# nttcslab-sp/torchain

Hardware: AMD Instinct MI355X
Metric: sequence-frames/sec through denominator fwd-bwd (higher is better)
Workload: dtype f32

## Files before the change

### torchain_amd/csrc/den_tied_device.h

```cpp
#pragma once

#include "den_device.h"

namespace tc {

namespace {

typedef float f4 __attribute__((ext_vector_type(4)));
typedef uint32_t u4 __attribute__((ext_vector_type(4)));
typedef __attribute__((address_space(3))) float lds_f;
typedef __attribute__((address_space(3))) uint32_t lds_u;
typedef __attribute__((address_space(3))) f4 lds_f4;
typedef __attribute__((address_space(3))) u4 lds_u4;

__device__ __forceinline__ float ldsf(uint32_t a) { return *reinterpret_cast<lds_f *>(a); }
__device__ __forceinline__ void ldsf_st(uint32_t a, float v) { *reinterpret_cast<lds_f *>(a) = v; }
__device__ __forceinline__ f4 lds4(uint32_t a) { return *reinterpret_cast<lds_f4 *>(a); }
__device__ __forceinline__ void lds4_st(uint32_t a, f4 v) { *reinterpret_cast<lds_f4 *>(a) = v; }
__device__ __forceinline__ void lds4_st_at(uint32_t base, uint32_t off, f4 v) {
  asm volatile("ds_write_b128 %0, %1 offset:%2" : : "v"(base), "v"(v), "i"(off) : "memory");
}
__device__ __forceinline__ u4 lds4u(uint32_t a) { return *reinterpret_cast<lds_u4 *>(a); }
__device__ __forceinline__ void lds_add_u32(uint32_t a, uint32_t v) {
  __hip_atomic_fetch_add(reinterpret_cast<lds_u *>(a), v, __ATOMIC_RELAXED, __HIP_MEMORY_SCOPE_WORKGROUP);
}

typedef __amdgpu_buffer_rsrc_t rsrc_t;
__device__ __forceinline__ rsrc_t make_rsrc(const void *ubase, uint32_t bytes) {
  return __builtin_amdgcn_make_buffer_rsrc(const_cast<void *>(ubase), 0, (int)bytes, 0x00020000);
}
__device__ __forceinline__ u4 bld4u(rsrc_t r, uint32_t voff, uint32_t soff) {
  return __builtin_amdgcn_raw_buffer_load_b128(r, (int)voff, (int)soff, 0);
}
__device__ __forceinline__ f4 bld4(rsrc_t r, uint32_t voff, uint32_t soff) {
  const u4 v = bld4u(r, voff, soff);
  return f4{__uint_as_float(v.x), __uint_as_float(v.y), __uint_as_float(v.z), __uint_as_float(v.w)};
}
template <int AUX>
__device__ __forceinline__ f4 bld4_aux(rsrc_t r, uint32_t voff, uint32_t soff) {
  const u4 v = __builtin_amdgcn_raw_buffer_load_b128(r, (int)voff, (int)soff, AUX);
  return f4{__uint_as_float(v.x), __uint_as_float(v.y), __uint_as_float(v.z), __uint_as_float(v.w)};
}
__device__ __forceinline__ void bst4(rsrc_t r, uint32_t voff, f4 v) {
#ifndef TC_STORE_AUX
#define TC_STORE_AUX 2
#endif
  __builtin_amdgcn_raw_buffer_store_b128(u4{__float_as_uint(v.x), __float_as_uint(v.y), __float_as_uint(v.z), __float_as_uint(v.w)},
                                         r, (int)voff, 0, TC_STORE_AUX);
}

template <int AUX>
__device__ __forceinline__ void bst4_aux(rsrc_t r, uint32_t voff, f4 v) {
  __builtin_amdgcn_raw_buffer_store_b128(u4{__float_as_uint(v.x), __float_as_uint(v.y), __float_as_uint(v.z), __float_as_uint(v.w)},
                                         r, (int)voff, 0, AUX);
}

__device__ __forceinline__ f4 mk4(float x) { return f4{x, x, x, x}; }
__device__ __forceinline__ float hsum(f4 v) { return (v.x + v.y) + (v.z + v.w); }
__device__ __forceinline__ float exp_med3(float x) { return __expf(__builtin_amdgcn_fmed3f(x, -30.0f, 30.0f)); }
__device__ __forceinline__ f4 exp4(f4 y) { return f4{exp_med3(y.x), exp_med3(y.y), exp_med3(y.z), exp_med3(y.w)}; }

__device__ __forceinline__ f4 row_ld(rsrc_t r, uint32_t voff, int vec) {
  if (vec) return bld4(r, voff, 0);
  return f4{__uint_as_float(__builtin_amdgcn_raw_buffer_load_b32(r, (int)voff, 0, 0)),
            __uint_as_float(__builtin_amdgcn_raw_buffer_load_b32(r, (int)voff, 4, 0)),
            __uint_as_float(__builtin_amdgcn_raw_buffer_load_b32(r, (int)voff, 8, 0)),
            __uint_as_float(__builtin_amdgcn_raw_buffer_load_b32(r, (int)voff, 12, 0))};
}
__device__ __forceinline__ void row_st(rsrc_t r, uint32_t voff, int vec, f4 v) {
  if (vec) {
    bst4(r, voff, v);
  } else {
    __builtin_amdgcn_raw_buffer_store_b32(__float_as_uint(v.x), r, (int)voff, 0, 0);
    __builtin_amdgcn_raw_buffer_store_b32(__float_as_uint(v.y), r, (int)voff, 4, 0);
    __builtin_amdgcn_raw_buffer_store_b32(__float_as_uint(v.z), r, (int)voff, 8, 0);
    __builtin_amdgcn_raw_buffer_store_b32(__float_as_uint(v.w), r, (int)voff, 12, 0);
  }
}

__device__ __forceinline__ float block_sum_a(float v, uint32_t red, int wave, uint32_t lane) {
  v = wave_sum(v);
  if (lane == 0) ldsf_st(red + 4u * (uint32_t)wave, v);
  __syncthreads();
  static_assert(kWaves == 16, "one DPP row holds the wave totals");
  float t = ldsf(red + 4u * (lane & 15u));
  t = dpp_add<0xB1>(t);
  t = dpp_add<0x4E>(t);
  t = dpp_add<0x124>(t);
  t = dpp_add<0x128>(t);
  return t;
}

__device__ __forceinline__ void gamma_add_a(uint32_t addr, float v) {
  int32_t q;
  asm("v_cvt_rpi_i32_f32 %0, %1" : "=v"(q) : "v"(v));
  lds_add_u32(addr, (uint32_t)q);
}

struct Chunk6 {
  u4 wa, wb, oc;
};

__device__ __forceinline__ void load_chunk(Chunk6 &q, rsrc_t stream, uint32_t lane16, int chunk) {
  const uint32_t so = (uint32_t)chunk * (3 * 64 * 16);
  q.wa = bld4u(stream, lane16, so);
  q.wb = bld4u(stream, lane16, so + 1024);
  q.oc = bld4u(stream, lane16, so + 2048);
}

__device__ __forceinline__ uint32_t lo16(uint32_t x) {
  uint32_t r;
  asm volatile("v_and_b32 %0, 0xffff, %1" : "=v"(r) : "v"(x));
  return r;
}
__device__ __forceinline__ uint32_t hi16(uint32_t x) {
  uint32_t r;
  asm volatile("v_lshrrev_b32 %0, 16, %1" : "=v"(r) : "v"(x));
  return r;
}

__device__ __forceinline__ uint32_t lo16w(uint32_t x) {
  uint32_t r;
  const uint32_t two = 2u;
  asm volatile("v_lshlrev_b32_sdwa %0, %1, %2 dst_sel:DWORD dst_unused:UNUSED_PAD src0_sel:DWORD src1_sel:WORD_0" : "=v"(r) : "s"(two), "v"(x));
  return r;
}
__device__ __forceinline__ uint32_t hi16w(uint32_t x) {
  uint32_t r;
  const uint32_t two = 2u;
  asm volatile("v_lshlrev_b32_sdwa %0, %1, %2 dst_sel:DWORD dst_unused:UNUSED_PAD src0_sel:DWORD src1_sel:WORD_1" : "=v"(r) : "s"(two), "v"(x));
  return r;
}

struct RowCommit {
  uint32_t row;
  uint32_t sec_row;
  int left;
  __device__ __forceinline__ void commit(float v) {
    asm volatile("s_mov_b32 m0, %1\n\ts_nop 0\n\tds_write_addtid_b32 %0" : : "v"(v), "s"(row) : "memory", "m0");
    --left;
    row = left == 0 ? sec_row : row + 256u;
  }
};

template <uint32_t SRC, int HALF>
__device__ __forceinline__ void do_chunk(const Chunk6 &q, uint32_t m, float &acc, RowCommit &rc) {
  uint32_t o[8];
  o[0] = lo16(q.oc.x);
  o[1] = hi16(q.oc.x);
  o[2] = lo16(q.oc.y);
  o[3] = hi16(q.oc.y);
  o[4] = lo16(q.oc.z);
  o[5] = hi16(q.oc.z);
  o[6] = lo16(q.oc.w);
  o[7] = hi16(q.oc.w);
  float a[8];
#pragma unroll
  for (int i = 0; i < 8; ++i) {
#ifdef TC_ABL_NOGATHER
    a[i] = __uint_as_float(o[i]);
#else
    a[i] = ldsf(SRC + o[i]);
#endif
  }
  const uint32_t w[8] = {q.wa.x, q.wa.y, q.wa.z, q.wa.w, q.wb.x, q.wb.y, q.wb.z, q.wb.w};
#pragma unroll
  for (int i = 0; i < 8; ++i) {
    acc = fmaf(a[i], __uint_as_float(w[i]), acc);
    const int bit = (i & 1) ? 4 * HALF + i / 2 : 8 + 4 * HALF + i / 2;
    if (__builtin_expect((m >> bit) & 1u, 0)) {
      rc.commit(acc);
      acc = 0.f;
    }
  }
}

__device__ __forceinline__ uint32_t wave_masks(const ScheduleDev &sc, int wave, uint32_t lane) {
  const uint32_t i = lane < (uint32_t)sc.mask_stride ? lane : (uint32_t)sc.mask_stride - 1u;
  return sc.masks[(size_t)wave * sc.mask_stride + i];
}

constexpr int kWalkEnd = -1000;

template <uint32_t SRC, int RES, class AfterChunk>
__device__ __forceinline__ void walk(const Chunk6 (&res)[RES > 0 ? RES : 1], Chunk6 &qa, rsrc_t sbase,
                                     uint32_t lane16, int nchunks, uint32_t vmask, RowCommit rc,
                                     AfterChunk after_chunk TC_WALK_ARG) {
  static_assert(RES % 2 == 0, "a mask word covers two chunks");
  auto mk = [&](int i) { return (uint32_t)__builtin_amdgcn_readlane((int)vmask, i); };
  float acc = 0.f;
#ifdef TC_PHASE_STAMPS
  wst[2] = clock64();
#endif
#pragma unroll
  for (int i = 0; i < RES / 2; ++i) {
    const uint32_t m = mk(i);
    do_chunk<SRC, 0>(res[2 * i], m, acc, rc);
    after_chunk(2 * i);
    do_chunk<SRC, 1>(res[2 * i + 1], m, acc, rc);
    after_chunk(2 * i + 1);
  }
#ifdef TC_PHASE_STAMPS
  {
    __builtin_amdgcn_s_waitcnt(0xC07F);
    const long long now = clock64();
    wst[0] += now - wst[2];
    wst[2] = now;
  }
#endif
  Chunk6 qb;
  int c = RES;
  for (; c + 2 < nchunks; c += 2) {
    const uint32_t m = mk(c >> 1);
    load_chunk(qb, sbase, lane16, c + 1);
    do_chunk<SRC, 0>(qa, m, acc, rc);
    load_chunk(qa, sbase, lane16, c + 2);
    do_chunk<SRC, 1>(qb, m, acc, rc);
    if (RES == 0) after_chunk(-1 - (c >> 1));
  }
  if (c + 1 < nchunks) {
    const uint32_t m = mk(c >> 1);
    load_chunk(qb, sbase, lane16, c + 1);
    do_chunk<SRC, 0>(qa, m, acc, rc);
    do_chunk<SRC, 1>(qb, m, acc, rc);
  } else if (c < nchunks) {
    do_chunk<SRC, 0>(qa, mk(c >> 1), acc, rc);
  }
  if (RES == 0) after_chunk(kWalkEnd);
#ifdef TC_PHASE_STAMPS
  __builtin_amdgcn_s_waitcnt(0xC07F);
  wst[1] += clock64() - wst[2];
#endif
}

template <uint32_t SRC>
__device__ __forceinline__ void chunk_pw(const Chunk6 &q, uint32_t m8, float &acc, RowCommit &rc) {
  uint32_t o[8];
  o[0] = lo16w(q.oc.x);
  o[1] = hi16w(q.oc.x);
  o[2] = lo16w(q.oc.y);
  o[3] = hi16w(q.oc.y);
  o[4] = lo16w(q.oc.z);
  o[5] = hi16w(q.oc.z);
  o[6] = lo16w(q.oc.w);
  o[7] = hi16w(q.oc.w);
  float a[8];
#pragma unroll
  for (int i = 0; i < 8; ++i) a[i] = ldsf(SRC + o[i]);
  const uint32_t w[8] = {q.wa.x, q.wa.y, q.wa.z, q.wa.w, q.wb.x, q.wb.y, q.wb.z, q.wb.w};
#pragma unroll
  for (int i = 0; i < 8; ++i) {
    acc = fmaf(a[i], __uint_as_float(w[i]), acc);
    if (__builtin_expect((m8 >> i) & 1u, 0)) {
      rc.commit(acc);
      acc = 0.f;
    }
  }
}

__device__ __forceinline__ void age_prio_on(int wave) {
  if (wave >= 12)
    __builtin_amdgcn_s_setprio(3);
  else if (wave >= 8)
    __builtin_amdgcn_s_setprio(2);
  else if (wave >= 4)
    __builtin_amdgcn_s_setprio(1);
}

__device__ __forceinline__ float tied_alpha(uint32_t pb, uint32_t fs, float ws, float F, float a_self) {
  return fmaf(ldsf(pb + (fs & 0xffffu)), F, ldsf(pb + (fs >> 16)) * (ws * a_self));
}

__device__ __forceinline__ f4 own_rows(uint32_t vrow, int j) {
  return f4{ldsf(vrow + 256u * (4 * j)), ldsf(vrow + 256u * (4 * j + 1)), ldsf(vrow + 256u * (4 * j + 2)),
            ldsf(vrow + 256u * (4 * j + 3))};
}

__device__ __forceinline__ void fold_row(int2 f, uint32_t vrow, uint32_t aACC, int Hs, int K) {
  const int k = 4 * (f.x / (4 * kThreads)) + (f.x & 3);
  const uint32_t dst = vrow + 256u * (uint32_t)k;
  const uint32_t src = aACC + 256u * (uint32_t)(K * kWaves) + 4u * (uint32_t)(f.y - Hs - 4);
  ldsf_st(dst, ldsf(dst) + ldsf(src));
}

__device__ __forceinline__ void fold_row_pw(int2 f, uint32_t vrow, uint32_t aACC, int Hs) {
  const uint32_t dst = vrow + 256u * (uint32_t)(f.x & 3);
  const uint32_t src = aACC + 256u * (uint32_t)(4 * kWaves) + 4u * (uint32_t)(f.y - Hs - 4);
  ldsf_st(dst, ldsf(dst) + ldsf(src));
}

constexpr uint32_t kPlane = 16u * kThreads;

struct AsumRow {
  uint32_t lds;
  float *g;
  __device__ __forceinline__ AsumRow(const DenParams &p, int s)
      : lds(4u * (uint32_t)p.L.off_asum), g(p.L.asum_global ? p.asum_g + (int64_t)s * asum_stride(p.T) : nullptr) {}
  __device__ __forceinline__ void st(int t, float v) const {
    if (g)
      g[t] = v;
    else
      ldsf_st(lds + 4u * (uint32_t)t, v);
  }
  __device__ __forceinline__ float ld(int t) const {
    if (g) return __uint_as_float(__builtin_amdgcn_raw_buffer_load_b32(make_rsrc(g + t, 4u), 0, 0, 0));
    return ldsf(lds + 4u * (uint32_t)t);
  }
};

}

#define TC_TIED_DISPATCH(CALL)                            \
  if (JV == kJvSmall && PV == kPvSmall) return CALL(kJvSmall, kPvSmall); \
  if (JV == kJvSmall && PV == kPvMid) return CALL(kJvSmall, kPvMid);     \
  if (JV == kJvSmall && PV == kPvLarge) return CALL(kJvSmall, kPvLarge); \
  if (JV == kJvMid && PV == kPvSmall) return CALL(kJvMid, kPvSmall);     \
  if (JV == kJvMid && PV == kPvMid) return CALL(kJvMid, kPvMid);         \
  if (JV == kJvMid && PV == kPvLarge) return CALL(kJvMid, kPvLarge);     \
  if (JV == kJvLarge && PV == kPvSmall) return CALL(kJvLarge, kPvSmall); \
  if (JV == kJvLarge && PV == kPvMid) return CALL(kJvLarge, kPvMid);     \
  if (JV == kJvLarge && PV == kPvLarge) return CALL(kJvLarge, kPvLarge);

}
```

### torchain_amd/csrc/den_tied_frames.h

```cpp
#pragma once

#include <type_traits>

#include "den_tied_device.h"

namespace tc {

__device__ __forceinline__ void block_sum2(float &v1, float &v2, uint32_t red, int wave, uint32_t lane) {
  v1 = wave_sum(v1);
  v2 = wave_sum(v2);
  if (lane == 0) {
    ldsf_st(red + 4u * (uint32_t)wave, v1);
    ldsf_st(red + 4u * (uint32_t)(kWaves + wave), v2);
  }
  __syncthreads();
  float t1 = ldsf(red + 4u * (lane & 15u)), t2 = ldsf(red + 4u * (kWaves + (lane & 15u)));
  t1 = dpp_add<0xB1>(t1);
  t2 = dpp_add<0xB1>(t2);
  t1 = dpp_add<0x4E>(t1);
  t2 = dpp_add<0x4E>(t2);
  t1 = dpp_add<0x124>(t1);
  t2 = dpp_add<0x124>(t2);
  v1 = dpp_add<0x128>(t1);
  v2 = dpp_add<0x128>(t2);
}

__device__ __forceinline__ float vload_f32(const float *ptr) {
  return __uint_as_float(__builtin_amdgcn_raw_buffer_load_b32(make_rsrc(ptr, 4u), 0, 0, 0));
}

template <bool GAMMA>
__device__ __forceinline__ float tied_fwd_state(uint32_t pb, uint32_t aGM, float inv_prev, uint32_t fsx, float wsx, float Fx, float alx,
                                                float bx, float gs, float &dpart) {
  const float pf = ldsf(pb + (fsx & 0xffffu)), ps = ldsf(pb + (fsx >> 16));
  const float sp = ps * (wsx * alx);
  const float a = fmaf(pf, Fx, sp) * inv_prev;
  if constexpr (GAMMA) {
    const float g = gs * bx, spn = sp * inv_prev;
    gamma_add_a(aGM + (fsx >> 16), g * spn);
    gamma_add_a(aGM + (fsx & 0xffffu), g * fmaxf(a - spn, 0.f));
    dpart = fmaf(a, bx, dpart);
  }
  return a;
}
template <bool PURE>
__device__ __forceinline__ float tied_bwd_state(uint32_t pb, uint32_t aGM, uint32_t fsx, float wsx, float bo, float alx, float aupx,
                                                float cpx, float ax, float inv_as, float asum_up) {
  const float ps_ws = ldsf(pb + (fsx >> 16)) * wsx;
  if constexpr (!PURE) {
    const float selfpart = ps_ws * alx * inv_as;
    const float bos = kGammaScale * bo;
    gamma_add_a(aGM + (fsx >> 16), bos * selfpart);
#ifndef TC_ABL_NOFADD
    gamma_add_a(aGM + (fsx & 0xffffu), bos * fmaxf((aupx - cpx * asum_up) - selfpart, 0.f));
#endif
  }
  return fmaf(ps_ws, bo, ax);
}

template <int JV, int PV, bool ALPHA_LDS, bool ACCUM, int RESF, int RESB, bool MITM>
struct TiedSeq {
  const DenParams &p;
  const uint32_t tid, lane;
  const int wave, s;
  const int H, P, S, T, Hs, Ps;
  const int planes, K;
  const uint32_t own16, lane16;
  static constexpr uint32_t kPB = 0u;
  static constexpr uint32_t kA0 = PV * 16u * kThreads;
  const uint32_t aACC;
  const uint32_t vrow;
  const uint32_t aGM;
  const uint32_t aAL;
  const uint32_t aRed, aAsum;
  const uint32_t tab_bytes, row_bytes;
  const rsrc_t r_pi, r_fs, r_ws;
  const float leaky;
  const int64_t hist_step;
  float *const hist;
  float *const fn;
  float *const bn;
  float *const bhist;
  const int M;

  int fnch, store_slot, bnch, bstore_slot;
  uint32_t fsec, bsec;
  uint32_t aFS, aWS;
  bool tabs_lds;
  uint32_t pb_cur, pb_next;
  rsrc_t fbase, bbase;
  float asum, inv_prev, bsum;
  float chat;
  float part, y2, part_tot;
  int ffx0, ffx1, bfx0, bfx1;
  uint32_t fmask, bmask;
  Chunk6 fres[RESF > 0 ? RESF : 1];
  Chunk6 bres[RESB > 0 ? RESB : 1];
  f4 v4[JV];
  f4 bt[JV];
  f4 areg[JV];
  f4 ycur[PV], ynext[PV];
  f4 bown[JV];
#ifdef TC_PHASE_STAMPS
  long long st_prev, st_acc[8];
#endif

  __device__ __forceinline__ TiedSeq(const DenParams &pp, int seq, int meet, int frames = 0)
      : p(pp), tid(threadIdx.x), lane(threadIdx.x & 63u), wave(__builtin_amdgcn_readfirstlane(threadIdx.x >> 6)), s(seq),
        H(pp.H), P(pp.P), S(pp.S), T(frames > 0 ? frames : pp.T), Hs(pp.L.Hs), Ps(pp.L.Ps), planes(pp.L.Hs / (4 * kThreads)), K(pp.L.Hs / kThreads),
        own16(16u * threadIdx.x), lane16(16u * (threadIdx.x & 63u)), aACC(4u * (uint32_t)pp.L.off_acc),
        vrow(4u * (uint32_t)pp.L.off_acc + 256u * (uint32_t)((pp.L.Hs / kThreads) * __builtin_amdgcn_readfirstlane(threadIdx.x >> 6)) +
             4u * (threadIdx.x & 63u)),
        aGM(4u * (uint32_t)pp.L.off_g), aAL(4u * (uint32_t)pp.L.off_al), aRed(4u * (uint32_t)pp.L.off_red),
        aAsum(4u * (uint32_t)pp.L.off_asum), tab_bytes(4u * (uint32_t)(pp.L.Hs + 4)), row_bytes(4u * (uint32_t)pp.P),
        r_pi(make_rsrc(pp.pi, 4u * (uint32_t)(pp.L.Hs + 4))), r_fs(make_rsrc(pp.tied_fs, 4u * (uint32_t)(pp.L.Hs + 4))),
        r_ws(make_rsrc(pp.tied_w, 4u * (uint32_t)(pp.L.Hs + 4))), leaky(pp.leaky), hist_step((int64_t)pp.S * pp.L.Hs),
        hist(pp.alpha_hist + (int64_t)seq * pp.L.Hs), fn(MITM ? pp.fwd_norm + (int64_t)seq * (pp.T + 2) : nullptr),
        bn(MITM ? pp.bwd_norm + (int64_t)seq * (pp.T + 1) : nullptr), bhist(MITM ? pp.beta_hist + (int64_t)seq * pp.L.Hs : nullptr),
        M(meet) {}

  __device__ __forceinline__ bool plane_on(int j) const { return j < planes; }

  __device__ __forceinline__ void stamps_reset() {
#ifdef TC_PHASE_STAMPS
    st_prev = clock64();
    for (int i = 0; i < 8; ++i) st_acc[i] = 0;
#endif
  }
  __device__ __forceinline__ void stamps_flush(int base) {
#ifdef TC_PHASE_STAMPS
    TC_STAMP(0)
    if (!MITM && blockIdx.x == 0 && lane == 0)
      for (int i = 0; i < 8; ++i) p.stamps[base + wave * 8 + i] = st_acc[i];
#endif
  }

  __device__ __forceinline__ void xent_zero_row(int t) {
    if (p.xent_zero) {
      const rsrc_t xrow = make_rsrc(p.xent_zero + ((int64_t)t * S + s) * p.xent_stride, row_bytes);
#pragma unroll
      for (int v = 0; v < PV; ++v)
        if (4 * ((int)tid + kThreads * v) < Ps) row_st(xrow, own16 + v * kPlane, p.x_vec, mk4(0.f));
    }
  }

  template <bool GAMMA>
  __device__ __forceinline__ float fwd_state(uint32_t fsx, float wsx, float Fx, float alx, float bx, float gs, float &dpart) {
    return tied_fwd_state<GAMMA>(kPB, aGM, inv_prev, fsx, wsx, Fx, alx, bx, gs, dpart);
  }
  template <bool PURE>
  __device__ __forceinline__ float bwd_state(uint32_t pb, uint32_t fsx, float wsx, float bo, float alx, float aupx, float cpx, float ax,
                                             float inv_as, float asum_up) {
    return tied_bwd_state<PURE>(pb, aGM, fsx, wsx, bo, alx, aupx, cpx, ax, inv_as, asum_up);
  }

  __device__ __forceinline__ void forward_begin() {
    f4 pi4[JV];
    part = 0.f;
#pragma unroll
    for (int j = 0; j < JV; ++j) {
      pi4[j] = plane_on(j) ? bld4(r_pi, own16, j * kPlane) : mk4(0.f);
      part += hsum(pi4[j]);
    }
    asum = block_sum_a(part, aRed, wave, lane);
#pragma unroll
    for (int j = 0; j < JV; ++j)
      if (plane_on(j)) {
        const f4 a = pi4[j] + (leaky * pi4[j]) * asum;
        lds4_st(kA0 + own16 + j * kPlane, a);
        bst4(make_rsrc(hist, 4u * Hs), own16 + j * kPlane, a);
      }
    y2 = 0.f;
    {
      const rsrc_t yrow = make_rsrc(p.y + (int64_t)s * p.y_stride, row_bytes);
#pragma unroll
      for (int v = 0; v < PV; ++v) {
        const int i0 = 4 * ((int)tid + kThreads * v);
        if (i0 < Ps) {
          const f4 yv = row_ld(yrow, own16 + v * kPlane, p.y_vec);
          y2 += hsum(yv * yv);
          lds4_st(kPB + 4u * i0, exp4(yv));
        }
      }
    }
    if (tid == 0) {
      ldsf_st(aAsum, asum);
      if (MITM) fn[0] = asum;
    }
    inv_prev = __builtin_amdgcn_rcpf(asum);

    {
    const int2 frange = p.fwd.wave_range[wave];
#ifdef TC_ABL_NOSTREAM
    fnch = RESF;
#else
    fnch = __builtin_amdgcn_readfirstlane(frange.y) / kChunk;
#endif
    fbase = make_rsrc(reinterpret_cast<const char *>(p.fwd.cells) +
                          (int64_t)(__builtin_amdgcn_readfirstlane(frange.x) / kChunk) * (3 * 64 * 16),
                      (uint32_t)(fnch + 2) * (3 * 64 * 16));
    fmask = wave_masks(p.fwd, wave, lane);
    ffx0 = p.fwd.nfix ? p.fwd.fix_begin[tid] : 0;
    ffx1 = p.fwd.nfix ? p.fwd.fix_begin[tid + 1] : 0;
    fsec = aACC + 256u * (uint32_t)(K * kWaves + p.fwd.extra_first[wave]);
#pragma unroll
    for (int i = 0; i < RESF; ++i) load_chunk(fres[i], fbase, lane16, i);
    }
    tabs_lds = (p.L.off_red - p.L.off_g) >= 2 * Hs;
    aFS = aGM;
    aWS = aGM + 4u * (uint32_t)Hs;
    if (tabs_lds) {
#pragma unroll
      for (int j = 0; j < JV; ++j)
        if (plane_on(j)) {
          *reinterpret_cast<lds_u4 *>(aFS + own16 + j * kPlane) = bld4u(r_fs, own16, j * kPlane);
          lds4_st(aWS + own16 + j * kPlane, bld4(r_ws, own16, j * kPlane));
        }
    }
    store_slot = RESF >= 4 ? wave >> 2 : RESF >= 2 ? wave >> 3 : 0;
#pragma unroll
    for (int j = 0; j < JV; ++j) v4[j] = bt[j] = mk4(0.f);
    chat = 0.f;
    part_tot = 0.f;
    stamps_reset();
  }

  static constexpr bool kHistFromPass = !MITM;

  template <bool GAMMA>
  __device__ __forceinline__ void forward_frame(int t) {
#ifdef TC_PHASE_STAMPS
    long long *const wst = st_acc + 5;
#endif
    TC_STAMP(0)
    Chunk6 q0;
    load_chunk(q0, fbase, lane16, RESF);
    __syncthreads();
    TC_STAMP(1)
    f4 yreg[PV];
    if (t < T) {
      const rsrc_t yrow = make_rsrc(p.y + ((int64_t)t * S + s) * p.y_stride, row_bytes);
#pragma unroll
      for (int v = 0; v < PV; ++v) yreg[v] = row_ld(yrow, own16 + v * kPlane, p.y_vec);
    }
    float n_t = 1.f;
    if (GAMMA && t < T) n_t = vload_f32(bn + t);
    age_prio_on(wave);
    bool stored = false;
    const RowCommit frc{aACC + 256u * (uint32_t)(K * wave), fsec, K};
    walk<kA0, RESF>(fres, q0, fbase, lane16, fnch, fmask, frc, [&](int i) {
      if (!kHistFromPass && !GAMMA && t > 1 && !stored && (RESF > 0 ? i == store_slot : (i == kWalkEnd || i == -1 - (wave >> 2)))) {
        stored = true;
        const rsrc_t hist_prev = make_rsrc(hist + (int64_t)(t - 1) * hist_step, 4u * Hs);
#ifndef TC_ABL_NOHIST
#pragma unroll
        for (int j = 0; j < JV; ++j)
          if (plane_on(j)) bst4(hist_prev, own16 + j * kPlane, lds4(kA0 + own16 + j * kPlane));
#endif
      }
    } TC_WALK_PASS);
    __builtin_amdgcn_s_setprio(0);
    TC_STAMP(2)
    for (int e = ffx0; e < ffx1; ++e) fold_row(p.fwd.fix[e], vrow, aACC, Hs, K);
    TC_STAMP(3)
    part = 0.f;
    float dpart = 0.f;
    u4 fs[JV];
    f4 ws[JV], cpi[JV];
#pragma unroll
    for (int j = 0; j < JV; ++j)
      if (plane_on(j)) {
        fs[j] = tabs_lds ? lds4u(aFS + own16 + j * kPlane) : bld4u(r_fs, own16, j * kPlane);
        ws[j] = tabs_lds ? lds4(aWS + own16 + j * kPlane) : bld4(r_ws, own16, j * kPlane);
        cpi[j] = bld4(r_pi, own16, j * kPlane);
      }
    const float gs = kGammaScale * chat;
    const rsrc_t hist_prev = make_rsrc(hist + (int64_t)(t - 1) * hist_step, t > 1 ? 4u * Hs : 0u);
#pragma unroll
    for (int j = 0; j < JV; ++j) {
      v4[j] = mk4(0.f);
      if (plane_on(j)) {
        const f4 F = own_rows(vrow, j);
        const f4 al = lds4(kA0 + own16 + j * kPlane);
#ifndef TC_ABL_NOHIST
        if (kHistFromPass && !GAMMA) bst4(hist_prev, own16 + j * kPlane, al);
#endif
        v4[j] = f4{fwd_state<GAMMA>(fs[j].x, ws[j].x, F.x, al.x, bt[j].x, gs, dpart), fwd_state<GAMMA>(fs[j].y, ws[j].y, F.y, al.y, bt[j].y, gs, dpart),
                   fwd_state<GAMMA>(fs[j].z, ws[j].z, F.z, al.z, bt[j].z, gs, dpart), fwd_state<GAMMA>(fs[j].w, ws[j].w, F.w, al.w, bt[j].w, gs, dpart)};
        part += hsum(v4[j]);
      }
    }
    f4 yp[PV];
    if (GAMMA) {
      const rsrc_t yprev = make_rsrc(p.y + ((int64_t)(t - 1) * S + s) * p.y_stride, row_bytes);
#pragma unroll
      for (int v = 0; v < PV; ++v) yp[v] = row_ld(yprev, own16 + v * kPlane, p.y_vec);
      const rsrc_t brow = make_rsrc(bhist + (int64_t)(t + 1 <= T ? t + 1 : T) * hist_step, 4u * Hs);
#pragma unroll
      for (int j = 0; j < JV; ++j) bt[j] = bld4(brow, own16, j * kPlane);
      block_sum2(part, dpart, aRed, wave, lane);
      asum = part;
    } else {
      asum = block_sum_a(part, aRed, wave, lane);
    }
    __builtin_amdgcn_sched_barrier(0);
    TC_STAMP(4)
    part_tot = 0.f;
#pragma unroll
    for (int j = 0; j < JV; ++j)
      if (plane_on(j)) {
        const f4 a = v4[j] + (leaky * cpi[j]) * asum;
        lds4_st(kA0 + own16 + j * kPlane, a);
        part_tot += hsum(a);
      }
    if (GAMMA) {
      const float c = __builtin_amdgcn_rcpf(dpart);
      const float sa = p.deriv_weight * (kGammaInvScale * (c * __builtin_amdgcn_rcpf(chat)));
      const rsrc_t drow = make_rsrc(p.deriv + ((int64_t)(t - 1) * S + s) * p.deriv_stride, row_bytes);
#pragma unroll
      for (int v = 0; v < PV; ++v) {
        const int i0 = 4 * ((int)tid + kThreads * v);
        if (i0 < Ps) {
          const u4 gu = lds4u(aGM + 4u * i0);
          lds4_st(aGM + 4u * i0, mk4(0.f));
          f4 o = sa * f4{(float)gu.x, (float)gu.y, (float)gu.z, (float)gu.w} - p.l2_scale * yp[v];
          if (ACCUM) o += row_ld(drow, own16 + v * kPlane, p.d_vec);
          row_st(drow, own16 + v * kPlane, p.d_vec, o);
        }
      }
      xent_zero_row(t - 1);
      chat = c * asum * __builtin_amdgcn_rcpf(n_t);
    }
    if (t < T) {
#pragma unroll
      for (int v = 0; v < PV; ++v) {
        const int i0 = 4 * ((int)tid + kThreads * v);
        if (i0 < Ps) {
          y2 += hsum(yreg[v] * yreg[v]);
          lds4_st(kPB + 4u * i0, exp4(yreg[v]));
        }
      }
    }
    if (tid == 0) {
      ldsf_st(aAsum + 4u * t, asum);
      if (MITM) fn[t] = asum;
    }
    inv_prev = __builtin_amdgcn_rcpf(asum);
  }

  __device__ __forceinline__ void forward_unpark() {
    tabs_lds = false;
#pragma unroll
    for (int v = 0; v < PV; ++v) {
      const int i0 = 4 * ((int)tid + kThreads * v);
      if (i0 < Ps) lds4_st(aGM + 4u * i0, mk4(0.f));
    }
  }

  __device__ __forceinline__ void forward_store_row(int t) {
    const rsrc_t hist_t = make_rsrc(hist + (int64_t)t * hist_step, 4u * Hs);
#pragma unroll
    for (int j = 0; j < JV; ++j)
      if (plane_on(j)) bst4(hist_t, own16 + j * kPlane, lds4(kA0 + own16 + j * kPlane));
  }

  __device__ __forceinline__ float forward_total(double bad) {
    const float tot = block_sum_a(part_tot, aRed + 4u * kWaves, wave, lane);
    const double y2d = (double)block_sum_a(y2, aRed + 8u * kWaves, wave, lane);
    if (tid == 0) {
      double logsum = 0.0;
      for (int t = 0; t < T; ++t) logsum += (double)__logf(ldsf(aAsum + 4u * t));
      p.seq_logprob[s] = logsum + (double)__logf(tot) + (y2d - y2d) + bad;
      p.seq_y2[s] = y2d;
    }
    return tot;
  }

  __device__ __forceinline__ void backward_store_row(int t) {
    const rsrc_t brow = make_rsrc(bhist + (int64_t)t * hist_step, 4u * Hs);
#pragma unroll
    for (int j = 0; j < JV; ++j)
      if (plane_on(j)) bst4(brow, own16 + j * kPlane, bown[j]);
  }

  template <bool PURE>
  __device__ __forceinline__ void backward_begin(float b_T) {
    part = 0.f;
#pragma unroll
    for (int j = 0; j < JV; ++j)
      if (plane_on(j)) part += hsum(leaky * bld4(r_pi, own16, j * kPlane)) * b_T;
    bsum = block_sum_a(part, aRed + 12u * kWaves, wave, lane);
    pb_cur = kPB;
    pb_next = ALPHA_LDS ? 4u * (uint32_t)p.L.off_p2 : kPB;
    {
    const int2 brange = p.bwd.wave_range[wave];
#ifdef TC_ABL_NOSTREAM
    bnch = RESB;
#else
    bnch = __builtin_amdgcn_readfirstlane(brange.y) / kChunk;
#endif
    bbase = make_rsrc(reinterpret_cast<const char *>(p.bwd.cells) +
                          (int64_t)(__builtin_amdgcn_readfirstlane(brange.x) / kChunk) * (3 * 64 * 16),
                      (uint32_t)(bnch + 2) * (3 * 64 * 16));
    bmask = wave_masks(p.bwd, wave, lane);
    bfx0 = p.bwd.nfix ? p.bwd.fix_begin[tid] : 0;
    bfx1 = p.bwd.nfix ? p.bwd.fix_begin[tid + 1] : 0;
    bsec = aACC + 256u * (uint32_t)(K * kWaves + p.bwd.extra_first[wave]);
#pragma unroll
    for (int i = 0; i < RESB; ++i) load_chunk(bres[i], bbase, lane16, i);
    }
    {
      const rsrc_t hist_up = make_rsrc(hist + (int64_t)T * hist_step, 4u * Hs);
      const rsrc_t bT = make_rsrc(bhist + (int64_t)T * hist_step, PURE ? 4u * Hs : 0u);
      const rsrc_t yrow = make_rsrc(p.y + ((int64_t)(T - 1) * S + s) * p.y_stride, row_bytes);
#pragma unroll
      for (int j = 0; j < JV; ++j) {
        bown[j] = areg[j] = mk4(0.f);
        if (plane_on(j)) {
          const int h0 = 4 * ((int)tid + kThreads * j);
          const float b = b_T + bsum;
          bown[j] = f4{h0 < H ? b : 0.f, h0 + 1 < H ? b : 0.f, h0 + 2 < H ? b : 0.f, h0 + 3 < H ? b : 0.f};
          if (PURE) bst4(bT, own16 + j * kPlane, bown[j]);
          if (!PURE && ALPHA_LDS) lds4_st(aAL + own16 + j * kPlane, bld4(hist_up, own16, j * kPlane));
        }
      }
#pragma unroll
      for (int v = 0; v < PV; ++v) {
        const int i0 = 4 * ((int)tid + kThreads * v);
        ycur[v] = row_ld(yrow, own16 + v * kPlane, p.y_vec);
        if (i0 < Ps) {
          lds4_st(pb_cur + 4u * i0, exp4(ycur[v]));
          lds4_st(aGM + 4u * i0, mk4(0.f));
        }
      }
      __syncthreads();
#pragma unroll
      for (int j = 0; j < JV; ++j)
        if (plane_on(j)) {
          const u4 fs = bld4u(r_fs, own16, j * kPlane);
          lds4_st(kA0 + own16 + j * kPlane,
                  f4{bown[j].x * ldsf(pb_cur + (fs.x & 0xffffu)), bown[j].y * ldsf(pb_cur + (fs.y & 0xffffu)),
                     bown[j].z * ldsf(pb_cur + (fs.z & 0xffffu)), bown[j].w * ldsf(pb_cur + (fs.w & 0xffffu))});
        }
    }
    bstore_slot = RESB >= 4 ? wave >> 2 : RESB >= 2 ? wave >> 3 : 0;
    stamps_reset();
  }

#ifdef TC_NO_BWD_DEFER
  static constexpr bool kDeferDeriv = false;
#else
  static constexpr bool kDeferDeriv = ALPHA_LDS;
#endif

  template <bool PURE>
  __device__ __forceinline__ bool backward_frame(int t, int t_top) {
#ifdef TC_PHASE_STAMPS
    long long *const wst = st_acc + 5;
#endif
    TC_STAMP(0)
    Chunk6 q0;
    load_chunk(q0, bbase, lane16, RESB);
    __syncthreads();
    TC_STAMP(1)
    const float asum_t = PURE ? 1.f : ldsf(aAsum + 4u * t);
    const float inv_as = __builtin_amdgcn_rcpf(asum_t);
    {
      const int tn = t > 0 ? t - 1 : 0;
      const rsrc_t yrow = make_rsrc(p.y + ((int64_t)tn * S + s) * p.y_stride, row_bytes);
#pragma unroll
#ifdef TC_ABL_NOY2
      for (int v = 0; v < PV; ++v) ynext[v] = mk4(0.25f) * (float)t;
#else
      for (int v = 0; v < PV; ++v) ynext[v] = row_ld(yrow, own16 + v * kPlane, p.y_vec);
#endif
      if (!PURE) {
        const rsrc_t hist_t = make_rsrc(hist + (int64_t)t * hist_step, 4u * Hs);
#pragma unroll
        for (int j = 0; j < JV; ++j) areg[j] = plane_on(j) ? bld4(hist_t, own16, j * kPlane) : mk4(0.f);
      }
    }
    age_prio_on(wave);
    bool dstored = false;
    const RowCommit brc{aACC + 256u * (uint32_t)(K * wave), bsec, K};
    walk<kA0, RESB>(bres, q0, bbase, lane16, bnch, bmask, brc, [&](int i) {
#ifndef TC_ABL_NOWALKSTORE
      if ((PURE ? t < T - 1 : kDeferDeriv && t < t_top - 1) && !dstored &&
          (RESB > 0 ? i == bstore_slot : (i == kWalkEnd || i == -1 - (wave >> 2)))) {
        dstored = true;
        if (PURE) {
          const rsrc_t brow_up = make_rsrc(bhist + (int64_t)(t + 1) * hist_step, 4u * Hs);
#pragma unroll
          for (int j = 0; j < JV; ++j)
            if (plane_on(j)) bst4(brow_up, own16 + j * kPlane, bown[j]);
        } else {
          const rsrc_t drow = make_rsrc(p.deriv + ((int64_t)(t + 1) * S + s) * p.deriv_stride, row_bytes);
#pragma unroll
          for (int v = 0; v < PV; ++v)
            if (4 * ((int)tid + kThreads * v) < Ps) row_st(drow, own16 + v * kPlane, p.d_vec, lds4(pb_next + own16 + v * kPlane));
          xent_zero_row(t + 1);
        }
      }
#endif
    } TC_WALK_PASS);
    __builtin_amdgcn_s_setprio(0);
    if (ALPHA_LDS) {
#pragma unroll
      for (int v = 0; v < PV; ++v) {
        const int i0 = 4 * ((int)tid + kThreads * v);
        if (i0 < Ps) lds4_st(pb_next + 4u * i0, exp4(ynext[v]));
      }
    }
    TC_STAMP(2)
    for (int e = bfx0; e < bfx1; ++e) fold_row(p.bwd.fix[e], vrow, aACC, Hs, K);
    TC_STAMP(3)
    f4 b4[JV];
    uint32_t fpk[JV][2];
    part = 0.f;
    float part_u = 0.f, part_ab = 0.f, part_g = 0.f;
    const float asum_up = PURE ? 0.f : ldsf(aAsum + 4u * (t + 1));
    constexpr bool kAhead = RESB == 0;
    u4 fs_n = u4{0u, 0u, 0u, 0u};
    f4 ws_n = mk4(0.f), cp_n = mk4(0.f), aup_n = mk4(0.f);
    auto request = [&](int j) __attribute__((always_inline)) {
      fs_n = bld4u(r_fs, own16, j * kPlane);
      ws_n = bld4(r_ws, own16, j * kPlane);
      cp_n = bld4(r_pi, own16, j * kPlane);
      if (!PURE && !ALPHA_LDS) aup_n = bld4(make_rsrc(hist + (int64_t)(t + 1) * hist_step, 4u * Hs), own16, j * kPlane);
    };
    if (kAhead) request(0);
#pragma unroll
    for (int j = 0; j < JV; ++j) {
      b4[j] = mk4(0.f);
      if (plane_on(j)) {
        if (!kAhead) request(j);
        const u4 fs = fs_n;
        const f4 ws = ws_n;
        const f4 cp = leaky * cp_n;
        const f4 aup_g = aup_n;
        if (kAhead && j + 1 < planes) request(j + 1);
        f4 a = own_rows(vrow, j);
        const f4 al = areg[j];
        const f4 aup = (!PURE && ALPHA_LDS) ? lds4(aAL + own16 + j * kPlane) : aup_g;
        a.x = bwd_state<PURE>(pb_cur, fs.x, ws.x, bown[j].x, al.x, aup.x, cp.x, a.x, inv_as, asum_up);
        a.y = bwd_state<PURE>(pb_cur, fs.y, ws.y, bown[j].y, al.y, aup.y, cp.y, a.y, inv_as, asum_up);
        a.z = bwd_state<PURE>(pb_cur, fs.z, ws.z, bown[j].z, al.z, aup.z, cp.z, a.z, inv_as, asum_up);
        a.w = bwd_state<PURE>(pb_cur, fs.w, ws.w, bown[j].w, al.w, aup.w, cp.w, a.w, inv_as, asum_up);
        b4[j] = PURE ? a : a * inv_as;
        fpk[j][0] = (fs.x & 0xffffu) | (fs.y << 16);
        fpk[j][1] = (fs.z & 0xffffu) | (fs.w << 16);
        part += hsum(cp * b4[j]);
        if (PURE) part_u += hsum(a);
        if (!PURE && t == 0) part_ab += hsum(al * b4[j]);
      }
    }
    float inv_n = 1.f;
    if (PURE) {
      block_sum2(part, part_u, aRed, wave, lane);
      const float n = part_u * (1.0f / (float)H);
      inv_n = __builtin_amdgcn_rcpf(n);
      bsum = part * inv_n;
      if (tid == 0) bn[t] = __builtin_amdgcn_rcpf(inv_n);
    } else {
      bsum = block_sum_a(part, aRed, wave, lane);
    }
    TC_STAMP(4)
    if (!PURE) {
      const rsrc_t drow = make_rsrc(p.deriv + ((int64_t)t * S + s) * p.deriv_stride, row_bytes);
#pragma unroll
      for (int v = 0; v < PV; ++v) {
        const int i0 = 4 * ((int)tid + kThreads * v);
        if (i0 < Ps) {
          const u4 gu = lds4u(aGM + 4u * i0);
          lds4_st(aGM + 4u * i0, mk4(0.f));
          const f4 g = f4{(float)gu.x, (float)gu.y, (float)gu.z, (float)gu.w} * kGammaInvScale;
          if (t == 0) part_g += hsum(g);
          f4 o = p.deriv_weight * g - p.l2_scale * ycur[v];
          if (ACCUM) o += row_ld(drow, own16 + v * kPlane, p.d_vec);
#ifndef TC_ABL_NODERIV
          if (kDeferDeriv && t > 0)
            lds4_st(pb_cur + 4u * i0, o);
          else
            row_st(drow, own16 + v * kPlane, p.d_vec, o);
#else
          if (o.x == 123.456f) row_st(drow, own16 + v * kPlane, p.d_vec, o);
#endif
        }
      }
      if (!(kDeferDeriv && t > 0)) xent_zero_row(t);
      if (t == 0) {
        const float ab = block_sum_a(part_ab, aRed + 4u * kWaves, wave, lane);
        const float gsum = block_sum_a(part_g, aRed + 8u * kWaves, wave, lane);
        if (tid == 0) {
          p.seq_ab[s] = ab;
          p.seq_gsum[s] = gsum;
        }
        return true;
      }
    }
    if (!ALPHA_LDS) {
#pragma unroll
      for (int v = 0; v < PV; ++v) {
        const int i0 = 4 * ((int)tid + kThreads * v);
        if (i0 < Ps) lds4_st(kPB + 4u * i0, exp4(ynext[v]));
      }
      __syncthreads();
    }
#pragma unroll
    for (int j = 0; j < JV; ++j)
      if (plane_on(j)) {
        const f4 b = PURE ? b4[j] * inv_n + bsum : b4[j] + bsum;
        bown[j] = b;
        const f4 yv = f4{b.x * ldsf(pb_next + (fpk[j][0] & 0xffffu)), b.y * ldsf(pb_next + (fpk[j][0] >> 16)),
                         b.z * ldsf(pb_next + (fpk[j][1] & 0xffffu)), b.w * ldsf(pb_next + (fpk[j][1] >> 16))};
        if constexpr (kA0 + (JV - 1) * kPlane < 65536u)
          lds4_st_at(own16, kA0 + j * kPlane, yv);
        else
          lds4_st(kA0 + own16 + j * kPlane, yv);
        if (!PURE && ALPHA_LDS) lds4_st(aAL + own16 + j * kPlane, areg[j]);
      }
#pragma unroll
    for (int v = 0; v < PV; ++v) ycur[v] = ynext[v];
    const uint32_t tmp = pb_cur;
    pb_cur = pb_next;
    pb_next = tmp;
    return false;
  }
};

}
```

Baseline: 28.81 million.

## Prefetch alpha history rows into LDS via buffer-load-to-LDS DMA in backward

Replaces the per-frame register load of the alpha history row plus the LDS park store with buffer_load ... lds instructions that write the next frame's row straight into LDS, one frame ahead. The current row is read from LDS, the previous row stays in registers, and a vmcnt wait with a computed depth orders the DMA against later loads. This aims to hide global-load latency and remove VGPR pressure and LDS store traffic. It adds inline asm that manipulates M0 and hand-counted vmcnt thresholds, which could be fragile.

```diff
diff --git a/torchain_amd/csrc/den_tied_device.h b/torchain_amd/csrc/den_tied_device.h
--- a/torchain_amd/csrc/den_tied_device.h
+++ b/torchain_amd/csrc/den_tied_device.h
@@ -54,6 +54,20 @@
   __builtin_amdgcn_raw_buffer_store_b128(u4{__float_as_uint(v.x), __float_as_uint(v.y), __float_as_uint(v.z), __float_as_uint(v.w)},
                                          r, (int)voff, 0, AUX);
 }
+
+__device__ __forceinline__ void dma4_to_lds(rsrc_t r, uint32_t voff, uint32_t lds_wave) {
+  uint32_t keep;
+  asm volatile("s_mov_b32 %0, m0\n\ts_mov_b32 m0, %3\n\ts_nop 4\n\tbuffer_load_dwordx4 %1, %2, 0 offen lds\n\ts_mov_b32 m0, %0"
+               : "=&s"(keep)
+               : "v"(voff), "s"(r), "s"(lds_wave)
+               : "memory");
+}
+template <int N>
+__device__ __forceinline__ void dma_wait() {
+  static_assert(N >= 0 && N < 64, "vmcnt is a 6-bit count");
+  asm volatile("s_waitcnt vmcnt(%0)" : : "n"(N) : "memory");
+}
+__device__ __forceinline__ void lds_wait_all() { asm volatile("s_waitcnt lgkmcnt(0)" : : : "memory"); }
 
 __device__ __forceinline__ f4 mk4(float x) { return f4{x, x, x, x}; }
 __device__ __forceinline__ float hsum(f4 v) { return (v.x + v.y) + (v.z + v.w); }
diff --git a/torchain_amd/csrc/den_tied_frames.h b/torchain_amd/csrc/den_tied_frames.h
--- a/torchain_amd/csrc/den_tied_frames.h
+++ b/torchain_amd/csrc/den_tied_frames.h
@@ -421,7 +421,12 @@
           const float b = b_T + bsum;
           bown[j] = f4{h0 < H ? b : 0.f, h0 + 1 < H ? b : 0.f, h0 + 2 < H ? b : 0.f, h0 + 3 < H ? b : 0.f};
           if (PURE) bst4(bT, own16 + j * kPlane, bown[j]);
-          if (!PURE && ALPHA_LDS) lds4_st(aAL + own16 + j * kPlane, bld4(hist_up, own16, j * kPlane));
+          if (!PURE && ALPHA_LDS) {
+            if (kHistByDma)
+              areg[j] = bld4(hist_up, own16, j * kPlane);
+            else
+              lds4_st(aAL + own16 + j * kPlane, bld4(hist_up, own16, j * kPlane));
+          }
         }
       }
 #pragma unroll
@@ -444,7 +449,26 @@
         }
     }
     bstore_slot = RESB >= 4 ? wave >> 2 : RESB >= 2 ? wave >> 3 : 0;
+    if (!PURE && kHistByDma) hist_dma(T - 1);
     stamps_reset();
+  }
+
+#ifdef TC_NO_HIST_DMA
+  static constexpr bool kHistByDma = false;
+#else
+  static constexpr bool kHistByDma = !MITM && ALPHA_LDS;
+#endif
+#ifdef TC_ABL_NOY2
+  static constexpr int kDmaBehind = 3;
+#else
+  static constexpr int kDmaBehind = 3 + PV;
+#endif
+
+  __device__ __forceinline__ void hist_dma(int t) {
+    const rsrc_t row = make_rsrc(hist + (int64_t)(t > 0 ? t : 0) * hist_step, t >= 0 ? 4u * Hs : 0u);
+#pragma unroll
+    for (int j = 0; j < JV; ++j)
+      if (plane_on(j)) dma4_to_lds(row, own16 + j * kPlane, aAL + 1024u * (uint32_t)wave + j * kPlane);
   }
 
 #ifdef TC_NO_BWD_DEFER
@@ -474,10 +498,14 @@
 #else
       for (int v = 0; v < PV; ++v) ynext[v] = row_ld(yrow, own16 + v * kPlane, p.y_vec);
 #endif
-      if (!PURE) {
+      if (!PURE && !kHistByDma) {
         const rsrc_t hist_t = make_rsrc(hist + (int64_t)t * hist_step, 4u * Hs);
 #pragma unroll
+#ifdef TC_ABL_NOHISTLOAD
+        for (int j = 0; j < JV; ++j) areg[j] = mk4(1e-4f) * (float)(t + 1);
+#else
         for (int j = 0; j < JV; ++j) areg[j] = plane_on(j) ? bld4(hist_t, own16, j * kPlane) : mk4(0.f);
+#endif
       }
     }
     age_prio_on(wave);
@@ -528,6 +556,7 @@
       cp_n = bld4(r_pi, own16, j * kPlane);
       if (!PURE && !ALPHA_LDS) aup_n = bld4(make_rsrc(hist + (int64_t)(t + 1) * hist_step, 4u * Hs), own16, j * kPlane);
     };
+    if (!PURE && kHistByDma) dma_wait<kDmaBehind>();
     if (kAhead) request(0);
 #pragma unroll
     for (int j = 0; j < JV; ++j) {
@@ -540,8 +569,9 @@
         const f4 aup_g = aup_n;
         if (kAhead && j + 1 < planes) request(j + 1);
         f4 a = own_rows(vrow, j);
-        const f4 al = areg[j];
-        const f4 aup = (!PURE && ALPHA_LDS) ? lds4(aAL + own16 + j * kPlane) : aup_g;
+        const f4 al = (!PURE && kHistByDma) ? lds4(aAL + own16 + j * kPlane) : areg[j];
+        const f4 aup = (!PURE && kHistByDma) ? areg[j] : (!PURE && ALPHA_LDS) ? lds4(aAL + own16 + j * kPlane) : aup_g;
+        if (!PURE && kHistByDma) areg[j] = al;
         a.x = bwd_state<PURE>(pb_cur, fs.x, ws.x, bown[j].x, al.x, aup.x, cp.x, a.x, inv_as, asum_up);
         a.y = bwd_state<PURE>(pb_cur, fs.y, ws.y, bown[j].y, al.y, aup.y, cp.y, a.y, inv_as, asum_up);
         a.z = bwd_state<PURE>(pb_cur, fs.z, ws.z, bown[j].z, al.z, aup.z, cp.z, a.z, inv_as, asum_up);
@@ -553,6 +583,10 @@
         if (PURE) part_u += hsum(a);
         if (!PURE && t == 0) part_ab += hsum(al * b4[j]);
       }
+    }
+    if (!PURE && kHistByDma) {
+      lds_wait_all();
+      hist_dma(t - 1);
     }
     float inv_n = 1.f;
     if (PURE) {
@@ -595,6 +629,7 @@
           p.seq_ab[s] = ab;
           p.seq_gsum[s] = gsum;
         }
+        if (kHistByDma) dma_wait<0>();
         return true;
       }
     }
@@ -617,7 +652,9 @@
           lds4_st_at(own16, kA0 + j * kPlane, yv);
         else
           lds4_st(kA0 + own16 + j * kPlane, yv);
-        if (!PURE && ALPHA_LDS) lds4_st(aAL + own16 + j * kPlane, areg[j]);
+#ifndef TC_ABL_NOPARK
+        if (!PURE && ALPHA_LDS && !kHistByDma) lds4_st(aAL + own16 + j * kPlane, areg[j]);
+#endif
       }
 #pragma unroll
     for (int v = 0; v < PV; ++v) ycur[v] = ynext[v];
```

After: 29.22 million (median of 6 runs). +1.4%, better.
